# sajadn/Exemplar-VAE

Measured on AMD Instinct MI355X. Metric: training images/sec, higher is better.
Workload: dtype f32

## Files before the change

exemplar-vae_amd/csrc/evae_dense.hip:

```cpp

#include "evae_gemm_x6.h"
#include "evae_gemm_p6.h"
#include "evae_thin.h"
#include "evae_u8_prepare.h"

namespace evae {

__global__ void gated_bwd_input_kernel(const float* __restrict__ dout, const float* __restrict__ gout,
                                       const float* __restrict__ s, int M, int N, int ldo,
                                       float* __restrict__ dh, float* __restrict__ dg, int ldd) {
  const size_t n = (size_t)M * N;
  size_t i = (size_t)blockIdx.x * blockDim.x + threadIdx.x;
  const size_t stride = (size_t)gridDim.x * blockDim.x;
  for (; i < n; i += stride) {
    const size_t row = i / N, col = i % N;
    const float d = dout[row * (size_t)ldd + col], ov = gout[i], sv = s[i];
    const size_t o = row * (size_t)ldo + col;
    dh[o] = d * sv;
    dg[o] = d * ov * (1.0f - sv);
  }
}

__global__ __launch_bounds__(256) void gated_bwd_input_v4_kernel(const float4* __restrict__ dout, const float4* __restrict__ gout,
                                                                 const float4* __restrict__ s, unsigned nquads, unsigned nq,
// ... 152 lines not shown
  g.out0 = (float*)ws; g.out1 = nullptr;
  int rc;
  if (gemm_x6_use(g)) {
    g.ksplit = pl.ksplit;
    rc = launch_gemm_x6<EPI_RAW>(g, pl.nz, stream, "linear_fwd(split-K, x6)");
  } else {
    rc = launch_gemm<true, true, EPI_RAW>(g, pl, stream, "linear_fwd(split-K)");
  }
  if (rc) return rc;
  FinishArgs f = {};
  f.ones_col = -1;
  f.part = (const float*)ws; f.nz = pl.nz; f.M = M; f.N = N; f.ldo = N; f.epi = EPI_LINEAR;
  f.bias0 = b; f.out0 = y; f.out1 = pre; f.act = act; f.lo = act_lo; f.hi = act_hi;
  return launch_finish(f, stream);
}

__global__ __launch_bounds__(256) void heads_reparam_finish_kernel(const float* __restrict__ part, int nz, int M, int Z,
                                                                   const float* __restrict__ bm, const float* __restrict__ bl,
                                                                   float lo, float hi, const float* __restrict__ eps,
                                                                   float* __restrict__ z_mean, float* __restrict__ lv_pre,
                                                                   float* __restrict__ logvar, float* __restrict__ z,
                                                                   float* __restrict__ logq, const float* __restrict__ z_given) {
  const int lane = threadIdx.x & 63;
  const int row = blockIdx.x * 4 + (threadIdx.x >> 6);
  if (row >= M) return;
  const size_t plane = (size_t)M * Z;
  float acc = 0.f;
  for (int k = lane; k < Z; k += 64) {
    const size_t o = (size_t)row * Z + k;
    float m = 0.f, p = 0.f;
    for (int s = 0; s < nz; ++s) { m += part[(size_t)s * 2 * plane + o]; p += part[(size_t)s * 2 * plane + plane + o]; }
    m += bm ? bm[k] : 0.f;
    p += bl ? bl[k] : 0.f;
    const float lv = fminf(fmaxf(p, lo), hi);
    const float zz = z_given ? z_given[o] : eps[o] * expf(0.5f * lv) + m;
    z_mean[o] = m;
    if (lv_pre) lv_pre[o] = p;
    logvar[o] = lv;
    if (!z_given) z[o] = zz;
    const float d = zz - m;
    acc += -0.5f * (lv + kLog2Pi + d * d / expf(lv));
  }
  acc = wave_sum(acc);
  if (lane == 0 && logq) logq[row] = acc;
}

static Plan heads_plan(int M, int K, int Z) { return make_plan(M, Z, cdiv(K, BK), true, true, 2); }

extern "C" size_t evae_heads_reparam_fwd_workspace_bytes(int M, int K, int Z) {
  if (M <= 0 || K <= 0 || Z <= 0) return 256;
  return align_up((size_t)heads_plan(M, K, Z).nz * 2 * M * Z * sizeof(float), 256) + 256;
}

static int heads_reparam_fwd_core(const float* x, int M, int K, int ldx, const float* wm, const float* bm, const float* wl,
                                  const float* bl, int Z, float lv_lo, float lv_hi, const float* eps, float* z_mean,
                                  float* lv_pre, float* logvar, float* z, float* logq, void* ws, size_t ws_bytes,
                                  const float* bc_src, float* bc_dst, int bc_n, evae_stream_t stream_);

extern "C" int evae_heads_reparam_fwd(const float* x, int M, int K, int ldx, const float* wm, const float* bm, const float* wl,
                                      const float* bl, int Z, float lv_lo, float lv_hi, const float* eps, float* z_mean,
                                      float* lv_pre, float* logvar, float* z, float* logq, void* ws, size_t ws_bytes,
                                      evae_stream_t stream_) {
  return heads_reparam_fwd_core(x, M, K, ldx, wm, bm, wl, bl, Z, lv_lo, lv_hi, eps, z_mean, lv_pre, logvar, z, logq, ws, ws_bytes,
                                nullptr, nullptr, 0, stream_);
}

extern "C" int evae_heads_reparam_fwd_bcast_applies(int M, int K, int Z, int ldx) {
  return M > 0 && thin_heads_ok(M, K, Z, ldx, nullptr, nullptr, nullptr) ? 1 : 0;
}
extern "C" int evae_heads_reparam_fwd_bcast(const float* x, int M, int K, int ldx, const float* wm, const float* bm, const float* wl,
                                            const float* bl, int Z, float lv_lo, float lv_hi, const float* eps, float* z_mean,
                                            float* lv_pre, float* logvar, float* z, float* logq, const float* src, float* dst,
                                            int n, evae_stream_t stream_) {
  EVAE_REQUIRE(src && dst && n > 0 && M > 0 && thin_heads_ok(M, K, Z, ldx, x, wm, wl), "heads_reparam_fwd_bcast: not the batch-sized case");
  return heads_reparam_fwd_core(x, M, K, ldx, wm, bm, wl, bl, Z, lv_lo, lv_hi, eps, z_mean, lv_pre, logvar, z, logq, nullptr, 0,
                                src, dst, n, stream_);
}

static int heads_reparam_fwd_core(const float* x, int M, int K, int ldx, const float* wm, const float* bm, const float* wl,
                                  const float* bl, int Z, float lv_lo, float lv_hi, const float* eps, float* z_mean,
                                  float* lv_pre, float* logvar, float* z, float* logq, void* ws, size_t ws_bytes,
                                  const float* bc_src, float* bc_dst, int bc_n, evae_stream_t stream_) {
  hipStream_t stream = (hipStream_t)stream_;
  EVAE_REQUIRE(M >= 0 && K > 0 && Z > 0 && ldx >= K, "heads_reparam_fwd: bad sizes M=%d K=%d Z=%d ldx=%d", M, K, Z, ldx);
  if (M == 0) return EVAE_OK;
  EVAE_REQUIRE(x && wm && wl && eps && z_mean && logvar && z, "heads_reparam_fwd: null pointer");
  if (thin_heads_ok(M, K, Z, ldx, x, wm, wl)) {
    const ThinHeadsArgs t = {x, ldx, M, K, Z, wm, bm, wl, bl, lv_lo, lv_hi, eps, nullptr, z_mean, lv_pre, logvar, z, logq, bc_src, bc_dst, bc_n};
    return launch_thin_heads(t, stream, "heads_reparam_fwd(thin)");
  }
  EVAE_REQUIRE(ws && ws_bytes >= evae_heads_reparam_fwd_workspace_bytes(M, K, Z), "heads_reparam_fwd: workspace too small (%zu)", ws_bytes);
  const Plan pl = heads_plan(M, K, Z);
  GemmArgs g = {};
  g.ones_col = -1;
  g.A[0] = x; g.B[0] = wm; g.Bg = wl; g.lda[0] = ldx; g.ldb[0] = K; g.Kc[0] = K; g.npairs = 1;
  g.M = M; g.N = Z; g.ldo = Z; g.out0 = (float*)ws;
  int rc = launch_gemm<true, true, EPI_RAW_GATED>(g, pl, stream, "heads_reparam_fwd(split-K)");
  if (rc) return rc;
  heads_reparam_finish_kernel<<<cdiv(M, 4), 256, 0, stream>>>((const float*)ws, pl.nz, M, Z, bm, bl, lv_lo, lv_hi, eps, z_mean,
                                                             lv_pre, logvar, z, logq, nullptr);
  return check_launch("heads_reparam_finish_kernel");
}

extern "C" int evae_heads_density_fwd(const float* x, int M, int K, int ldx, const float* wm, const float* bm, const float* wl,
                                      const float* bl, int Z, float lv_lo, float lv_hi, const float* zq, float* z_mean, float* lv_pre,
                                      float* logvar, float* logp, void* ws, size_t ws_bytes, evae_stream_t stream_) {
  hipStream_t stream = (hipStream_t)stream_;
  EVAE_REQUIRE(M >= 0 && K > 0 && Z > 0 && ldx >= K, "heads_density_fwd: bad sizes M=%d K=%d Z=%d ldx=%d", M, K, Z, ldx);
  if (M == 0) return EVAE_OK;
  EVAE_REQUIRE(x && wm && wl && zq && z_mean && logvar && logp, "heads_density_fwd: null pointer");
  if (thin_heads_ok(M, K, Z, ldx, x, wm, wl)) {
    const ThinHeadsArgs t = {x, ldx, M, K, Z, wm, bm, wl, bl, lv_lo, lv_hi, nullptr, zq, z_mean, lv_pre, logvar, nullptr, logp};
    return launch_thin_heads(t, stream, "heads_density_fwd(thin)");
  }
  EVAE_REQUIRE(ws && ws_bytes >= evae_heads_reparam_fwd_workspace_bytes(M, K, Z), "heads_density_fwd: workspace too small (%zu)", ws_bytes);
  const Plan pl = heads_plan(M, K, Z);
  GemmArgs g = {};
  g.ones_col = -1;
  g.A[0] = x; g.B[0] = wm; g.Bg = wl; g.lda[0] = ldx; g.ldb[0] = K; g.Kc[0] = K; g.npairs = 1;
  g.M = M; g.N = Z; g.ldo = Z; g.out0 = (float*)ws;
  int rc = launch_gemm<true, true, EPI_RAW_GATED>(g, pl, stream, "heads_density_fwd(split-K)");
  if (rc) return rc;
  heads_reparam_finish_kernel<<<cdiv(M, 4), 256, 0, stream>>>((const float*)ws, pl.nz, M, Z, bm, bl, lv_lo, lv_hi, nullptr, z_mean,
                                                             lv_pre, logvar, nullptr, logp, zq);
  return check_launch("heads_density_finish");
}

static int x6_wt_ld(int N) { return (N + 3) / 4 * 4; }
static size_t x6_wt_bytes(int N, int K, int npairs) { return align_up((size_t)npairs * K * x6_wt_ld(N) * sizeof(float), 256); }

__global__ __launch_bounds__(256) void transpose_pairs_kernel(const float* __restrict__ w1, const float* __restrict__ w2, int N,
                                                              int K, int ldt, float* __restrict__ wT) {
  __shared__ float tile[32][33];
  const float* w = blockIdx.z ? w2 : w1;
  float* o = wT + (size_t)blockIdx.z * K * ldt;
  const int n0 = blockIdx.y * 32, k0 = blockIdx.x * 32, tx = threadIdx.x & 31, ty = threadIdx.x >> 5;
  for (int r = ty; r < 32; r += 8)
    tile[r][tx] = (n0 + r < N && k0 + tx < K) ? w[(size_t)(n0 + r) * K + k0 + tx] : 0.f;
  __syncthreads();
  for (int r = ty; r < 32; r += 8)
    if (k0 + r < K && n0 + tx < ldt) o[(size_t)(k0 + r) * ldt + n0 + tx] = tile[tx][r];
}

extern "C" size_t evae_dense_bwd_data_workspace_bytes(int M, int N, int K, int npairs) {
  if (M <= 0 || K <= 0 || N <= 0) return 256;
  Plan pl = make_plan(M, K, total_slabs(N, npairs > 1 ? N : 0), false, false, 1);
  const size_t wt = x6_wt_bytes(N, K, npairs > 1 ? 2 : 1);
  if (pl.nz <= 1) return 256 + wt;
  return align_up((size_t)pl.nz * M * K * sizeof(float), 256) + wt + 256;
}

struct ImgSink { unsigned short* img; int nslab, mbase; };

static int dense_bwd_data_core(const float* dy1, const float* w1, const float* dy2, const float* w2,
                               int M, int N, int ldy, int K, const float* out_prev, const float* s_prev,
                               float* dx_or_dh, float* dg, int ldo, const float* wT_ext, void* ws, size_t ws_bytes,
                               evae_stream_t stream_, const ImgSink* sink = nullptr, const P6Sink* tsink = nullptr) {
  hipStream_t stream = (hipStream_t)stream_;
  EVAE_REQUIRE(M >= 0 && N > 0 && K > 0 && ldy >= N && (sink || (tsink && !dx_or_dh) || ldo >= K), "dense_bwd_data: bad sizes M=%d N=%d K=%d", M, N, K);
  if (M == 0) return EVAE_OK;
  EVAE_REQUIRE(dy1 && w1 && (dx_or_dh || sink || tsink), "dense_bwd_data: null pointer");
  EVAE_REQUIRE((dy2 == nullptr) == (w2 == nullptr), "dense_bwd_data: dy2/w2 must come together");
  const bool gate = out_prev != nullptr;
  EVAE_REQUIRE(!gate || (s_prev && (dg || sink || (tsink && !dx_or_dh))), "dense_bwd_data: gate fusion needs out_prev, s_prev and dg");
  EVAE_REQUIRE(!tsink || gate, "dense_bwd_data: the transposed-image output comes with the gate epilogue only");
  const int np = dy2 ? 2 : 1;
  if (thin_ok(M, N, ldy, dy1, dy2) && (!sink || (sink->mbase % 8) == 0)) {
    ThinArgs t = {};
    t.A = dy1; t.A1 = dy2; t.lda = ldy; t.W0 = w1; t.W1 = w2; t.M = M; t.N = N; t.K = K;
    t.out0 = dx_or_dh; t.out1 = gate ? dg : nullptr; t.ldo = ldo; t.e0 = out_prev; t.e1 = s_prev;
    if (tsink) t.tsink = *tsink;
    if (sink) { t.u8img = sink->img; t.u8_nslab = sink->nslab; t.u8_mbase = sink->mbase; }
    if (gate) return launch_thin<THIN_GATE_BWD, true>(t, (hipStream_t)stream_, "dense_bwd_data(thin, gate)");
    return launch_thin<THIN_LINEAR, true>(t, (hipStream_t)stream_, "dense_bwd_data(thin)");
  }
  Plan pl = make_plan(M, K, total_slabs(N, np > 1 ? N : 0), false, false, 1);
  if (sink) { pl.nz = 1; pl.ksplit = 0; }
  GemmArgs g = {};
  if (sink) { g.img = sink->img; g.img_nslab = sink->nslab; g.img_mbase = sink->mbase; }
  if (tsink) g.tsink = *tsink;
  g.ones_col = -1;
  g.A[0] = dy1; g.B[0] = w1; g.lda[0] = ldy; g.ldb[0] = K; g.Kc[0] = N; g.npairs = np;
  if (dy2) { g.A[1] = dy2; g.B[1] = w2; g.lda[1] = ldy; g.ldb[1] = K; g.Kc[1] = N; }
  g.M = M; g.N = K; g.out0 = dx_or_dh; g.out1 = gate ? dg : nullptr; g.ldo = ldo; g.e0 = out_prev; g.e1 = s_prev;
  const size_t part_bytes = pl.nz > 1 ? align_up((size_t)pl.nz * M * K * sizeof(float), 256) : 0;
  const bool x6 = gemm_x6_enabled() && gemm_x6_fills(M, K, false) && ws && ws_bytes >= part_bytes + x6_wt_bytes(N, K, np) &&
                  N % 4 == 0 && ldy % 4 == 0 && (((uintptr_t)dy1 | (uintptr_t)dy2) & 15) == 0 && (long long)M * ldy < (1ll << 29);
  if (x6) {
    const int ldt = x6_wt_ld(N);
    const float* wT = wT_ext;
    if (wT == nullptr) {
      float* wTw = (float*)((char*)ws + part_bytes);
      transpose_pairs_kernel<<<dim3(cdiv(K, 32), cdiv(ldt, 32), np), 256, 0, stream>>>(w1, w2, N, K, ldt, wTw);
      int rc = check_launch("transpose_pairs_kernel");
      if (rc) return rc;
      wT = wTw;
    }
    g.B[0] = wT; g.ldb[0] = ldt;
    if (dy2) { g.B[1] = wT + (size_t)K * ldt; g.ldb[1] = ldt; }
  }
  if (pl.nz <= 1) {
    const bool narrow = x6 && gemm_x6_pick_bn(M, K) == 64;
    if (sink) {
      if (x6 && narrow) return launch_gemm_x6<EPI_GATE_BWD_IMG, 0, 64>(g, 1, stream, "dense_bwd_data(gate, bf16 tile images, x6)");
      if (x6) return launch_gemm_x6<EPI_GATE_BWD_IMG>(g, 1, stream, "dense_bwd_data(gate, bf16 tile images, x6)");
      return launch_gemm<true, false, EPI_GATE_BWD_IMG>(g, pl, stream, "dense_bwd_data(gate, bf16 tile images)");
    }
    if (x6 && gate && narrow) return launch_gemm_x6<EPI_GATE_BWD, 0, 64>(g, 1, stream, "dense_bwd_data(gate, x6)");
    if (x6 && gate) return launch_gemm_x6<EPI_GATE_BWD>(g, 1, stream, "dense_bwd_data(gate, x6)");
    if (x6 && narrow) return launch_gemm_x6<EPI_LINEAR, 0, 64>(g, 1, stream, "dense_bwd_data(x6)");
    if (x6) return launch_gemm_x6<EPI_LINEAR>(g, 1, stream, "dense_bwd_data(x6)");
    if (gate) return launch_gemm<true, false, EPI_GATE_BWD>(g, pl, stream, "dense_bwd_data(gate)");
    return launch_gemm<true, false, EPI_LINEAR>(g, pl, stream, "dense_bwd_data");
  }
  if (ws == nullptr || ws_bytes < part_bytes + 256) {
    set_error("dense_bwd_data: workspace too small (%zu)", ws_bytes);
    return EVAE_EWORKSPACE;
  }
  g.out0 = (float*)ws; g.out1 = nullptr;
  int rc;
  if (x6) {
    g.ksplit = pl.ksplit;
    rc = launch_gemm_x6<EPI_RAW>(g, pl.nz, stream, "dense_bwd_data(split-K, x6)");
  } else {
    rc = launch_gemm<true, false, EPI_RAW>(g, pl, stream, "dense_bwd_data(split-K)");
  }
  if (rc) return rc;
  FinishArgs f = {};
  f.ones_col = -1;
  f.part = (const float*)ws; f.nz = pl.nz; f.M = M; f.N = K; f.ldo = ldo;
  f.epi = gate ? EPI_GATE_BWD : EPI_LINEAR; f.out0 = dx_or_dh; f.out1 = gate ? dg : nullptr;
  f.e0 = out_prev; f.e1 = s_prev;
  if (tsink) f.tsink = *tsink;
  return launch_finish(f, stream);
}

extern "C" int evae_dense_bwd_data(const float* dy1, const float* w1, const float* dy2, const float* w2,
                                   int M, int N, int ldy, int K, const float* out_prev, const float* s_prev,
                                   float* dx_or_dh, float* dg, int ldo, void* ws, size_t ws_bytes,
                                   evae_stream_t stream_) {
  return dense_bwd_data_core(dy1, w1, dy2, w2, M, N, ldy, K, out_prev, s_prev, dx_or_dh, dg, ldo, nullptr, ws, ws_bytes, stream_);
}

extern "C" size_t evae_dense_bwd_data_wt_bytes(int N, int K, int npairs) {
  return (N > 0 && K > 0) ? x6_wt_bytes(N, K, npairs > 1 ? 2 : 1) : 0;
}
extern "C" int evae_dense_bwd_data_wt_ld(int N) { return x6_wt_ld(N); }

extern "C" int evae_dense_bwd_data_wt(const float* dy1, const float* w1, const float* dy2, const float* w2,
                                      int M, int N, int ldy, int K, const float* out_prev, const float* s_prev,
                                      float* dx_or_dh, float* dg, int ldo, const float* wT, void* ws, size_t ws_bytes,
                                      evae_stream_t stream_) {
  return dense_bwd_data_core(dy1, w1, dy2, w2, M, N, ldy, K, out_prev, s_prev, dx_or_dh, dg, ldo, wT, ws, ws_bytes, stream_);
}

extern "C" int evae_dense_bwd_data_timg(const float* dy1, const float* w1, const float* dy2, const float* w2,
                                        int M, int N, int ldy, int K, const float* out_prev, const float* s_prev,
                                        float* dx_or_dh, float* dg, int ldo, const float* wT, void* timg, int t_nks, int t_row0,
                                        int t_kbase, void* ws, size_t ws_bytes, evae_stream_t stream_) {
  EVAE_REQUIRE(timg && t_nks > 0 && t_row0 >= 0 && t_kbase >= 0 && (t_kbase % 8) == 0 && (t_kbase + M + 15) / 16 <= t_nks,
               "dense_bwd_data_timg: bad image placement (k-steps %d, first k %d, rows %d)", t_nks, t_kbase, M);
  const P6Sink sink = {(unsigned char*)timg, t_nks, t_row0, t_kbase, t_kbase + M};
  return dense_bwd_data_core(dy1, w1, dy2, w2, M, N, ldy, K, out_prev, s_prev, dx_or_dh, dg, ldo, wT, ws, ws_bytes, stream_, nullptr,
                             &sink);
}

extern "C" int evae_dense_bwd_data_img(const float* dy1, const float* w1, const float* dy2, const float* w2, int M, int N,
                                       int ldy, int K, const float* out_prev, const float* s_prev, void* img, int img_nslab,
                                       int m_base, const float* wT, void* ws, size_t ws_bytes, evae_stream_t stream_) {
  EVAE_REQUIRE(M >= 0 && N > 0 && K > 0 && ldy >= N, "dense_bwd_data_img: bad sizes M=%d N=%d K=%d", M, N, K);
  if (M == 0) return EVAE_OK;
  EVAE_REQUIRE(dy1 && w1 && out_prev && s_prev && img, "dense_bwd_data_img: null pointer");
  EVAE_REQUIRE(m_base % 8 == 0 && m_base >= 0 && img_nslab > 0 && (long long)m_base + M <= (long long)img_nslab * 32,
               "dense_bwd_data_img: the launch's first image row must be a multiple of 8 inside the image (M=%d m_base=%d nslab=%d)",
               M, m_base, img_nslab);
  const ImgSink sink = {(unsigned short*)img, img_nslab, m_base};
  return dense_bwd_data_core(dy1, w1, dy2, w2, M, N, ldy, K, out_prev, s_prev, nullptr, nullptr, K, wT, ws, ws_bytes, stream_, &sink);
}


__global__ __launch_bounds__(256) void narrow_wgrad_kernel(const float* __restrict__ dy, int ldy, const float* __restrict__ x,
                                                           int ldx, int M, int N, int K, int rows_per_slice,
                                                           float* __restrict__ part) {
  __shared__ float4 sdy[2][32][16];
  __shared__ float4 sx[2][32][16];
  const int Kp = K + 1;
  const int k0 = blockIdx.x * 64, z = blockIdx.y;
  const int r_begin = z * rows_per_slice, r_end = min(M, r_begin + rows_per_slice);
  const int tid = threadIdx.x, kg = tid & 15, ng = tid >> 4;
  const bool live = 4 * ng < N;
  float acc[4][4];
#pragma unroll
  for (int i = 0; i < 4; ++i)
#pragma unroll
    for (int j = 0; j < 4; ++j) acc[i][j] = 0.f;
  const int c4 = tid & 15, rr0 = tid >> 4;
  const bool dy_col = 4 * c4 < N;
  const int kx = k0 + 4 * c4;
  const bool x_vec = kx + 3 < K;
  float4 vd[2], vx[2];
  auto fetch = [&](int r0) {
#pragma unroll
    for (int it = 0; it < 2; ++it) {
      const int r = r0 + rr0 + 16 * it;
      vd[it] = make_float4(0.f, 0.f, 0.f, 0.f); vx[it] = vd[it];
      if (r < r_end) {
        if (dy_col) vd[it] = *reinterpret_cast<const float4*>(dy + (size_t)r * ldy + 4 * c4);
        if (x_vec) {
          vx[it] = *reinterpret_cast<const float4*>(x + (size_t)r * ldx + kx);
        } else {
          float t[4];
#pragma unroll
          for (int j = 0; j < 4; ++j) t[j] = (kx + j < K) ? x[(size_t)r * ldx + kx + j] : (kx + j == K ? 1.f : 0.f);
          vx[it] = make_float4(t[0], t[1], t[2], t[3]);
        }
      }
    }
  };
  auto stage = [&](int buf) {
#pragma unroll
    for (int it = 0; it < 2; ++it) { sdy[buf][rr0 + 16 * it][c4] = vd[it]; sx[buf][rr0 + 16 * it][c4] = vx[it]; }
  };
  fetch(r_begin);
  stage(0);
  __syncthreads();
  int buf = 0;
  for (int r0 = r_begin; r0 < r_end; r0 += 32, buf ^= 1) {
    const bool more = r0 + 32 < r_end;
// ... 527 lines not shown
```

exemplar-vae_amd/evae/fused_vae.py:

```python
import ctypes as C
import os

import torch
import torch.distributed as dist

from . import _lib, handoff, ops, shard

ACT_NONE, ACT_SIGMOID, ACT_HARDTANH = ops.ACT_NONE, ops.ACT_SIGMOID, ops.ACT_HARDTANH

_STAGE_GEN = {}
_XT_GEN = {}
_ZEROED = {}
def node_merge(Cl, B):
    e = os.environ.get("EVAE_NODE_MERGE")
    if e is not None:
        return int(e)
    return 15 if Cl + B <= 8192 else 11


ONE_STREAM = [os.environ.get("EVAE_ONE_STREAM", "0") == "1"]
_APPROX_ROWS = {}

SCHED = int(os.environ.get("EVAE_SCHED", "0"))
FINISH_GROUP_HEAD = os.environ.get("EVAE_FINISH_GROUP_HEAD", "0") == "1"
# ... 591 lines not shown
        with torch.cuda.stream(side):
            if not dpx_done:
                _lib.check(lib.evae_bernoulli_sigmoid_bwd(_vp(x), _vp(xmean), _vp(cRE), B, D, _vp(dpx), kd.st), "bernoulli_sigmoid_bwd")
            kd.bwd_data(dpx, wp, None, None, B, D, D, H, D2, sd2, dp2, dp2.data_ptr() + 4 * H, 2 * H)
            kd.bwd_data(dp2, d2h, dp2.data_ptr() + 4 * H, d2g, B, H, 2 * H, H, D1, sd1, dp1, dp1.data_ptr() + 4 * H, 2 * H)
            kd.bwd_data(dp1, d1h, dp1.data_ptr() + 4 * H, d1g, B, H, 2 * H, Z, None, None, dz, None, Z)
            side.wait_event(dz_ready)
            if prior_finish is not None:
                prior_finish()
            NODE_MERGE = node_merge(Cl, B)
            if NODE_MERGE & 12:
                RE_, logq_, logp_, loss_, KL_, means_ = ctx.elbo_keep if prior_done else (None,) * 6
                if prior_done and not (NODE_MERGE & 4):
                    _lib.check(lib.evae_elbo_assemble(_vp(logp_), _vp(RE_), _vp(logq_), _vp(beta_dev), 0.0 if beta_dev is not None else float(beta),
                                                      B, _vp(loss_), _vp(KL_), _vp(means_), kd.st), "elbo_assemble")
                    loss_ = None
                sum_here = bool(NODE_MERGE & 8)
                _lib.check(lib.evae_reparam_logq_bwd_hardtanh_tail(
                    _vp(z_mean), _vp(logvar), _vp(eps), _vp(z), _vp(dz), _vp(dzp), _vp(cKL), _vp(lv_pre), -6.0, 2.0, B, Z,
                    _vp(dmean_all.data_ptr() + off * Z), _vp(dlvp), _vp(logp_), _vp(RE_), _vp(logq_), _vp(beta_dev),
                    0.0 if beta_dev is not None else float(beta), _vp(loss_), _vp(KL_), _vp(means_),
                    _vp(dlv) if sum_here else None, Z, _vp(g_plv) if sum_here else None, kd.st), "reparam_bwd_tail")
            else:
                if prior_done:
                    RE_, logq_, logp_, loss_, KL_, means_ = ctx.elbo_keep
                    _lib.check(lib.evae_elbo_assemble(_vp(logp_), _vp(RE_), _vp(logq_), _vp(beta_dev), 0.0 if beta_dev is not None else float(beta),
                                                      B, _vp(loss_), _vp(KL_), _vp(means_), kd.st), "elbo_assemble")
                _lib.check(lib.evae_reparam_logq_bwd_hardtanh(_vp(z_mean), _vp(logvar), _vp(eps), _vp(z), _vp(dz), _vp(dzp), _vp(cKL),
                                                              _vp(lv_pre), -6.0, 2.0, B, Z, _vp(dmean_all.data_ptr() + off * Z),
                                                              _vp(dlvp), kd.st), "reparam_bwd")
            if headw_early:
                kd.bwd_weight(dmean_all, Mp, Z, Z, A2, None, H, H, g_wm, g_bm)
            if p6:
                nbh = lib.evae_dense_bwd_data_workspace_bytes(B, Z, H, 2)
                wh2 = kd.ws("dgrad", nbh)
                _lib.check(lib.evae_dense_bwd_data_timg(_vp(dmean_all.data_ptr() + off * Z), _vp(wm), _vp(dlvp), _vp(wl), B, Z, Z, H,
                                                        _vp(A2.data_ptr() + off * H), _vp(s2.data_ptr() + off * H),
                                                        _vp(dq2.data_ptr() + off * 2 * H), _vp(dq2.data_ptr() + off * 2 * H + 4 * H), 2 * H,
                                                        None, _vp(t_dq2), nks_m, 0, Cl, _vp(wh2), wh2.numel(), kd.st), "bwd_data_timg(batch)")
            else:
                kd.bwd_data(dmean_all.data_ptr() + off * Z, wm, dlvp, wl, B, Z, Z, H, A2.data_ptr() + off * H,
                            s2.data_ptr() + off * H, dq2.data_ptr() + off * 2 * H, dq2.data_ptr() + off * 2 * H + 4 * H, 2 * H)
            dq2_rows_done = torch.cuda.Event(); dq2_rows_done.record()
            l2_dgrad(kd, B, off, Cl)
            batch_rows_done.record()


        def leaves():
            with torch.cuda.stream(side):
                if fin_group and FINISH_GROUP_HEAD:
                    kd.bwd_weight(dmean_all, Mp, Z, Z, A2, None, H, H, g_wm, g_bm, phase=1, ws_name="wgradh")
                elif not headw_early:
                    kd.bwd_weight(dmean_all, Mp, Z, Z, A2, None, H, H, g_wm, g_bm)
                jobs = ((dpx, B, D, D, D2, H, H, g_wp, g_bp), (dp2, B, 2 * H, 2 * H, D1, H, H, g_d2, g_e2),
                        (dp1, B, 2 * H, 2 * H, z, Z, Z, g_d1, g_e1),
                        (dlvp, B, Z, Z, A2.data_ptr() + off * H, H, H, g_wl, g_bl))
                grouped = B <= 128 and GROUP_LEAVES and all(n_ % 4 == 0 and k_ % 4 == 0 for _, _, n_, _, _, k_, _, _, _ in jobs)
                if grouped:
                    arr = (_lib.WgradJob * len(jobs))()
                    for i_, (dy_, m_, n_, ldy_, x_, k_, ldx_, dw_, db_) in enumerate(jobs):
                        arr[i_].dy = dy_.data_ptr(); arr[i_].x = x_ if isinstance(x_, int) else x_.data_ptr()
                        arr[i_].dw = dw_.data_ptr(); arr[i_].db = db_.data_ptr()
                        arr[i_].M, arr[i_].N, arr[i_].K, arr[i_].ldy, arr[i_].ldx = m_, n_, k_, ldy_, ldx_
                    _lib.check(lib.evae_dense_bwd_weight_group(C.cast(arr, C.c_void_p), len(jobs), kd.st), "bwd_weight_group")
                else:
                    for dy_, m_, n_, ldy_, x_, k_, ldx_, dw_, db_ in jobs:
                        kd.bwd_weight(dy_, m_, n_, ldy_, x_, None, k_, ldx_, dw_, db_)
                if not (NODE_MERGE & 8):
                    _lib.check(lib.evae_sum_small(_vp(dlv), Z, _vp(g_plv), kd.st), "sum_small")
        leaves()
        split_wait = bool(SCHED & 256) and not (SCHED & 10)
        main.wait_event(dq2_rows_done if split_wait else batch_rows_done)
        g_w2 = gslot("w2", 2 * H, H); g_b2 = gslot("b2", 2 * H)
        w2_args = (dq2, Mp, 2 * H, 2 * H, A1, None, H, H, g_w2, g_b2)
        g_w1 = gslot("w1", 2 * H, D); g_b1 = gslot("b1", 2 * H)
        def w1_grad(no_finish=False):
            if data_ext.dtype == torch.uint8:
                nb = lib.evae_dense_bwd_weight_u8_workspace_bytes(Mp, 2 * H, D)
                w = k.ws("wgrad_u8_fused", nb)
                fl = 2.0 * Mp * 2 * H * D
                have_xt = ctx.xt is not None and ctx.xt == (w.data_ptr(), _XT_GEN.get(w.data_ptr()))
                ops.probed("dense_bwd_weight_u8 M=%d N=%d K=%d (uint8 rows, three bf16 terms; %s)"
                           % (Mp, 2 * H, D, "GEMM; planes summed by the step's last grouped launch" if no_finish else "pre-passes + GEMM + finish"),
                           fl, lambda: _lib.check(lib.evae_dense_bwd_weight_u8_phased(_vp(dq1), Mp, 2 * H, 2 * H, _vp(data_ext), _vp(rows), D,
                                                                                      ldd, 1.0 / 255.0, _vp(g_w1), _vp(g_b1), _vp(w),
                                                                                      w.numel(), (4 if have_xt else 0) | (16 if no_finish else 0), k.st)
                                              if (have_xt or no_finish) else
                                              lib.evae_dense_bwd_weight_u8(_vp(dq1), Mp, 2 * H, 2 * H, _vp(data_ext), _vp(rows), D,
                                                                           ldd, 1.0 / 255.0, _vp(g_w1), _vp(g_b1), _vp(w),
                                                                           w.numel(), k.st), "bwd_weight_u8"),
                           executed=3 * fl, pipe="bf16-mfma")
            else:
                k.bwd_weight(dq1, Mp, 2 * H, 2 * H, data_ext, rows, D, ldd, g_w1, g_b1)
        if SCHED & 2:
            k.bwd_weight(*w2_args, phase=1, ws_name="wgrad2")
            w2_done = torch.cuda.Event(); w2_done.record()
            w1_grad()
            with torch.cuda.stream(side):
                side.wait_event(w2_done)
                k.bwd_weight(*w2_args, phase=2, ws_name="wgrad2", finish_on=kd)
        elif (SCHED & 8) and data_ext.dtype == torch.uint8:
            nb = lib.evae_dense_bwd_weight_u8_workspace_bytes(Mp, 2 * H, D)
            w = k.ws("wgrad_u8_fused", nb)

            def w1_phase(phase, st):
                _lib.check(lib.evae_dense_bwd_weight_u8_phased(_vp(dq1), Mp, 2 * H, 2 * H, _vp(data_ext), _vp(rows), D, ldd, 1.0 / 255.0,
                                                               _vp(g_w1), _vp(g_b1), _vp(w), w.numel(), phase, st), "bwd_weight_u8_phased")
            dq1_ready = torch.cuda.Event(); dq1_ready.record()
            with torch.cuda.stream(side):
                side.wait_event(dq1_ready)
                w1_phase(1, kd.st)
                pre_done = torch.cuda.Event(); pre_done.record()
            k.bwd_weight(*w2_args)
            main.wait_event(pre_done)
            w1_phase(2, k.st)
        elif fin_group:
            k.bwd_weight(*w2_args, phase=1, ws_name="wgrad2")
            if split_wait:
                main.wait_event(batch_rows_done)
            w1_grad(no_finish=True)
            if FINISH_GROUP_HEAD:
                main.wait_stream(side)
            arr = (_lib.WgradFinishJob * 3)()
            w_u8 = k.ws("wgrad_u8_fused", lib.evae_dense_bwd_weight_u8_workspace_bytes(Mp, 2 * H, D))
            w_2 = ops._workspace("wgrad2" + k.sfx, lib.evae_dense_bwd_weight_workspace_bytes(Mp, 2 * H, H), dev)
            w_h = ops._workspace("wgradh" + kd.sfx, lib.evae_dense_bwd_weight_workspace_bytes(Mp, Z, H), dev)
            fjobs = ((1, Mp, 2 * H, D, 2 * H, ldd, 1.0 / 255.0, g_w1, g_b1, w_u8), (0, Mp, 2 * H, H, 2 * H, H, 1.0, g_w2, g_b2, w_2),
                     (0, Mp, Z, H, Z, H, 1.0, g_wm, g_bm, w_h))[:3 if FINISH_GROUP_HEAD else 2]
            for i_, (byte_, m_, n_, k_, ldy_, ldx_, xs_, dw_, db_, ws_) in enumerate(fjobs):
                arr[i_].byte_rows, arr[i_].M, arr[i_].N, arr[i_].K, arr[i_].ldy, arr[i_].ldx = byte_, m_, n_, k_, ldy_, ldx_
                arr[i_].x_scale = xs_; arr[i_].dw = dw_.data_ptr(); arr[i_].db = db_.data_ptr()
                arr[i_].ws = ws_.data_ptr(); arr[i_].ws_bytes = ws_.numel()
            _lib.check(lib.evae_dense_bwd_weight_finish_group(C.cast(arr, C.c_void_p), len(fjobs), k.st), "bwd_weight_finish_group")
        elif p6:
            nbw = lib.evae_dense_bwd_weight_p6_workspace_bytes(nks_m, 2 * H, H)
            ww = k.ws("wgrad_p6", nbw)
            flw = 2.0 * Mp * 2 * H * H
            ops.probed("dense_bwd_weight M=%d N=%d K=%d (+db; pre-split bf16 images, split-K GEMM + finish)" % (Mp, 2 * H, H), flw,
                       lambda: _lib.check(lib.evae_dense_bwd_weight_p6(_vp(t_dq2), _vp(t_h1), nks_m, 2 * H, H, _vp(g_w2), _vp(g_b2), _vp(ww),
                                                                       ww.numel(), k.st), "bwd_weight_p6"), executed=6 * flw, pipe="bf16-mfma")
            if split_wait:
                main.wait_event(batch_rows_done)
            w1_grad()
        else:
            k.bwd_weight(*w2_args)
            if split_wait:
                main.wait_event(batch_rows_done)
            w1_grad()
        main.wait_stream(side)
        ctx.bufs = None
        ctx.elbo_keep = None
        ctx.prior_done = None
        ctx.dd = None
        grads = (g_plv, g_wp, g_bp, g_w1[:H], g_b1[:H], g_w1[H:], g_b1[H:], g_w2[:H], g_b2[:H], g_w2[H:], g_b2[H:],
                 g_wm, g_bm, g_wl, g_bl, g_d1[:H], g_e1[:H], g_d1[H:], g_e1[H:], g_d2[:H], g_e2[:H], g_d2[H:], g_e2[H:])
        return (None,) * 15 + grads
```

Measured before the change: 185,800.

## Add streaming MFMA kernel for small-Z gated head data-gradient

Adds a specialised kernel for the backward data GEMM when the inner dimension is small (N<=64) with a gate epilogue. Each block stages a chunk of gate activations into LDS with vectorized loads, does the tiny GEMM with f32 MFMA from register-held dy rows, then applies the gating epilogue and optionally writes the split bf16 image. It replaces the general tiled GEMM path for these head-layer shapes, which is meant to cut launch and tiling overhead for a memory-bound op. It adds LDS-heavy blocks sized to the CU count, and it frees two ctx references in Python.

```diff
diff --git a/exemplar-vae_amd/csrc/evae_dense.hip b/exemplar-vae_amd/csrc/evae_dense.hip
--- a/exemplar-vae_amd/csrc/evae_dense.hip
+++ b/exemplar-vae_amd/csrc/evae_dense.hip
@@ -328,6 +328,148 @@
 
 struct ImgSink { unsigned short* img; int nslab, mbase; };
 
+constexpr int HS_ROWS = 32;
+constexpr int HS_NT = 512;
+constexpr int HS_TPW = 5;
+constexpr int HS_STAGE = 3;
+
+template <int ZS>
+__global__ __launch_bounds__(HS_NT, 4) void head_dgrad_stream_kernel(const float* __restrict__ dy, int ldy, const float* __restrict__ w,
+                                                                  int M, int Z, int N, const float* __restrict__ e0,
+                                                                  const float* __restrict__ e1, float* __restrict__ out0,
+                                                                  float* __restrict__ out1, int ldo, const P6Sink sink,
+                                                                  int rows_per_block) {
+  typedef float f32x4 __attribute__((ext_vector_type(4)));
+  extern __shared__ float4 hs_smem[];
+  float4* const sgo4 = hs_smem;
+  float4* const ssv4 = hs_smem + HS_ROWS * N / 4;
+  const float* const sgo = reinterpret_cast<const float*>(sgo4);
+  const float* const ssv = reinterpret_cast<const float*>(ssv4);
+  const int wv = threadIdx.x >> 6, l = threadIdx.x & 63, q = l >> 4, j = l & 15;
+  const int rbeg = blockIdx.x * rows_per_block, rend = min(M, rbeg + rows_per_block);
+  const int row0 = sink.img ? sink.row0 : 0;
+  const int g0 = row0 >> 4, ngrp = ((row0 + 2 * N + 15) >> 4) - g0;
+  for (int mc = rbeg; mc < rend; mc += HS_ROWS) {
+    const int nr = min(HS_ROWS, rend - mc);
+    float a[2][ZS];
+#pragma unroll
+    for (int T = 0; T < 2; ++T) {
+      const int m = mc + 8 * (j >> 2) + 4 * T + (j & 3);
+#pragma unroll
+      for (int s = 0; s < ZS; ++s) a[T][s] = (m < rend && 4 * s + q < Z) ? dy[(size_t)m * ldy + 4 * s + q] : 0.f;
+    }
+    const size_t base = (size_t)mc * N;
+    const int cnt = nr * N, nv = cnt >> 2;
+    const float4* const p0 = reinterpret_cast<const float4*>(e0 + base);
+    const float4* const p1 = reinterpret_cast<const float4*>(e1 + base);
+    for (int i0 = threadIdx.x; i0 < nv; i0 += HS_STAGE * HS_NT) {
+      float4 r0[HS_STAGE], r1[HS_STAGE];
+#pragma unroll
+      for (int u = 0; u < HS_STAGE; ++u) {
+        const int i = i0 + u * HS_NT;
+        if (i < nv) { r0[u] = p0[i]; r1[u] = p1[i]; }
+      }
+#pragma unroll
+      for (int u = 0; u < HS_STAGE; ++u) {
+        const int i = i0 + u * HS_NT;
+        if (i < nv) { sgo4[i] = r0[u]; ssv4[i] = r1[u]; }
+      }
+    }
+    if ((int)threadIdx.x < cnt - 4 * nv) {
+      const int i = 4 * nv + threadIdx.x;
+      reinterpret_cast<float*>(sgo4)[i] = e0[base + i];
+      reinterpret_cast<float*>(ssv4)[i] = e1[base + i];
+    }
+    __syncthreads();
+#pragma unroll 1
+    for (int t = 0; wv + 8 * t < ngrp; ++t) {
+      const int c = 16 * (g0 + wv + 8 * t) + j - row0;
+      const bool cok = c >= 0 && c < 2 * N, isg = c >= N;
+      const int n = cok ? (isg ? c - N : c) : 0;
+      float bw[ZS];
+#pragma unroll
+      for (int s = 0; s < ZS; ++s) bw[s] = (cok && 4 * s + q < Z) ? w[(4 * s + q) * N + n] : 0.f;
+      f32x4 acc0 = {0.f, 0.f, 0.f, 0.f}, acc1 = {0.f, 0.f, 0.f, 0.f};
+#pragma unroll
+      for (int s = 0; s < ZS; ++s) {
+        acc0 = __builtin_amdgcn_mfma_f32_16x16x4f32(a[0][s], bw[s], acc0, 0, 0, 0);
+        acc1 = __builtin_amdgcn_mfma_f32_16x16x4f32(a[1][s], bw[s], acc1, 0, 0, 0);
+      }
+      float go[8], sv[8];
+#pragma unroll
+      for (int i = 0; i < 8; ++i) {
+        const int ml = 8 * q + i;
+        const bool ok = cok && ml < nr;
+        go[i] = ok ? sgo[ml * N + n] : 0.f;
+        sv[i] = ok ? ssv[ml * N + n] : 0.f;
+      }
+      float o[8];
+#pragma unroll
+      for (int i = 0; i < 8; ++i) {
+        const float v = i < 4 ? acc0[i & 3] : acc1[i & 3];
+        const bool ok = cok && 8 * q + i < nr;
+        o[i] = ok ? (isg ? v * go[i] * (1.0f - sv[i]) : v * sv[i]) : 0.f;
+        if (ok && out0) (isg ? out1 : out0)[(size_t)(mc + 8 * q + i) * ldo + n] = o[i];
+      }
+      if (sink.img && cok && 8 * q < nr) {
+        uint4 p[3];
+        p6_split2(o[0], o[1], p[0].x, p[1].x, p[2].x);
+        p6_split2(o[2], o[3], p[0].y, p[1].y, p[2].y);
+        p6_split2(o[4], o[5], p[0].z, p[1].z, p[2].z);
+        p6_split2(o[6], o[7], p[0].w, p[1].w, p[2].w);
+        unsigned char* const dst = sink.img + p6_off(16 * (g0 + wv + 8 * t) + j, sink.kbase + mc + 8 * q, sink.nks);
+#pragma unroll
+        for (int pl = 0; pl < 3; ++pl) *reinterpret_cast<uint4*>(dst + pl * P6_CHUNK) = p[pl];
+      }
+    }
+    if (mc + HS_ROWS < rend) __syncthreads();
+  }
+}
+
+static size_t head_stream_lds(int N) { return 2 * ((size_t)HS_ROWS * N / 4) * sizeof(float4); }
+
+static bool head_stream_enabled() { const char* e = getenv("EVAE_DGRAD_STREAM"); return !(e && atoi(e) == 0); }
+
+static int device_cus() {
+  static int n = 0;
+  if (n <= 0) {
+    int d = 0;
+    if (hipGetDevice(&d) != hipSuccess || hipDeviceGetAttribute(&n, hipDeviceAttributeMultiprocessorCount, d) != hipSuccess || n <= 0) n = 256;
+  }
+  return n;
+}
+
+static bool head_stream_shape(int N, int K, const float* dy2, const float* out_prev, const float* s_prev, const P6Sink* tsink) {
+  if (dy2 || !out_prev || !s_prev || N > 64) return false;
+  const int row0 = tsink ? tsink->row0 : 0;
+  if (((row0 + 2 * K + 15) >> 4) - (row0 >> 4) > 8 * HS_TPW) return false;
+  return (((uintptr_t)out_prev | (uintptr_t)s_prev) & 15) == 0;
+}
+
+static int launch_head_stream(const float* dy, int ldy, const float* w, int M, int N, int K, const float* out_prev, const float* s_prev,
+                              float* dh, float* dg, int ldo, const P6Sink* tsink, hipStream_t stream) {
+  P6Sink sink = {};
+  if (tsink) sink = *tsink;
+  const int rpb = (int)align_up((size_t)cdiv(M, 2 * device_cus()), 8), nb = cdiv(M, rpb);
+  const size_t lds = head_stream_lds(K);
+  const int zs = cdiv(N, 4);
+#define EVAE_HS_LAUNCH(ZS_)                                                                                                        \
+  do {                                                                                                                             \
+    static bool attr = false;                                                                                                      \
+    if (!attr) {                                                                                                                   \
+      (void)hipFuncSetAttribute((const void*)head_dgrad_stream_kernel<ZS_>, hipFuncAttributeMaxDynamicSharedMemorySize,            \
+                                (int)head_stream_lds(64 * HS_TPW));                                                                \
+      attr = true;                                                                                                                 \
+    }                                                                                                                              \
+    head_dgrad_stream_kernel<ZS_><<<nb, HS_NT, lds, stream>>>(dy, ldy, w, M, N, K, out_prev, s_prev, dh, dg, ldo, sink, rpb);      \
+  } while (0)
+  if (zs <= 4) EVAE_HS_LAUNCH(4);
+  else if (zs <= 10) EVAE_HS_LAUNCH(10);
+  else EVAE_HS_LAUNCH(16);
+#undef EVAE_HS_LAUNCH
+  return check_launch("head_dgrad_stream_kernel");
+}
+
 static int dense_bwd_data_core(const float* dy1, const float* w1, const float* dy2, const float* w2,
                                int M, int N, int ldy, int K, const float* out_prev, const float* s_prev,
                                float* dx_or_dh, float* dg, int ldo, const float* wT_ext, void* ws, size_t ws_bytes,
@@ -350,6 +492,8 @@
     if (gate) return launch_thin<THIN_GATE_BWD, true>(t, (hipStream_t)stream_, "dense_bwd_data(thin, gate)");
     return launch_thin<THIN_LINEAR, true>(t, (hipStream_t)stream_, "dense_bwd_data(thin)");
   }
+  if (!sink && head_stream_enabled() && head_stream_shape(N, K, dy2, out_prev, s_prev, tsink))
+    return launch_head_stream(dy1, ldy, w1, M, N, K, out_prev, s_prev, dx_or_dh, dg, ldo, tsink, stream);
   Plan pl = make_plan(M, K, total_slabs(N, np > 1 ? N : 0), false, false, 1);
   if (sink) { pl.nz = 1; pl.ksplit = 0; }
   GemmArgs g = {};
diff --git a/exemplar-vae_amd/evae/fused_vae.py b/exemplar-vae_amd/evae/fused_vae.py
--- a/exemplar-vae_amd/evae/fused_vae.py
+++ b/exemplar-vae_amd/evae/fused_vae.py
@@ -767,6 +767,7 @@
         ctx.elbo_keep = None
         ctx.prior_done = None
         ctx.dd = None
+        ctx.dpx = None; ctx.coef = None
         grads = (g_plv, g_wp, g_bp, g_w1[:H], g_b1[:H], g_w1[H:], g_b1[H:], g_w2[:H], g_b2[:H], g_w2[H:], g_b2[H:],
                  g_wm, g_bm, g_wl, g_bl, g_d1[:H], g_e1[:H], g_d1[H:], g_e1[H:], g_d2[:H], g_e2[:H], g_d2[H:], g_e2[H:])
         return (None,) * 15 + grads
```

Result: slower. 180,800 (-2.7%).
